# apple/ml-fastvlm

Hardware: AMD Instinct MI355X
Metric: images/sec FastViTHD encode_images @1024x1024 bf16 (higher is better)
Workload: dtype bf16; 1 GPU; BASELINE.json configs[1]: FastViTHD encoder + mlp2x_gelu projector (H=896), batch=32/GPU synthetic 1024x1024 bf16 images in [0,1), seeded synthetic weights, single GPU; global_batch=32, image_size=1024, parallelism=dp1, hip_graph=False, attention_operands=bf16, ffn_precision=auto (calibrated on the benchmark batch), range guard on

## Files before the change

### ml_fastvlm_amd/csrc/gemm.hip

```cpp
#include "fvhd_common.h"
#include "launchers.h"
#include "gemm_layout.h"
#include "rope.h"
#include <stdlib.h>

#define EPI_NONE 0
#define EPI_BIAS 1
#define EPI_BIAS_GELU 2
#define EPI_BIAS_LS_RESID 3
#define EPI_RESID 4
static_assert(FVHD_EPI_SWIGLU_ID == 5 && FVHD_ODT_BF16_ID == FVHD_BF16, "gemm_layout.h ids");
#define EPI_SWIGLU 5

#define EPI_BIAS_ROPE 6

struct RopeArgs {
    const long* pos; const float* table; bf16* kcache; bf16* vcache;
    int M, T, nh, nkv, P; float theta;
};

template <int BK>
FVHD_DEV int lds_off(int row, int ks)
{
    if constexpr (BK == 64) return row * 128 + ((ks ^ ((row >> 1) & 7)) << 4);
    else return row * 64 + ((ks ^ ((0 - (row >> 2)) & 3)) << 4);
}

template <int MF, int NF, int EPI, int ODT, bool ROWMAJOR_ = false>
FVHD_DEV void gemm_epilogue(f32x4 (&acc)[MF][NF], const float* __restrict__ bias, const float* __restrict__ ls, const bf16* resid, void* out,
                            int M, int N, int mw, int nw, int lr, int g)
{
    constexpr int GRP = EpiGrp<NF, EPI, ODT>::value;
#if defined(FVHD_GEMM_EPI_COLMAJOR)
    constexpr bool ROWMAJOR = false;
#elif defined(FVHD_GEMM_EPI_ROWMAJOR)
    constexpr bool ROWMAJOR = ROWMAJOR_;
#else
    constexpr bool ROWMAJOR = ROWMAJOR_ && EPI == EPI_NONE;
#endif
    if constexpr (GRP == 1) {
#pragma unroll
        for (int j = 0; j < NF; ++j) {
            const int n = nw + j * 16 + g * 4;
            if (n >= N) continue;
            f32x4 bv = f32x4{0.f, 0.f, 0.f, 0.f}, lv = f32x4{1.f, 1.f, 1.f, 1.f};
            if constexpr (EPI == EPI_BIAS || EPI == EPI_BIAS_GELU || EPI == EPI_BIAS_LS_RESID) bv = *(const f32x4*)(bias + n);
            if constexpr (EPI == EPI_BIAS_LS_RESID) lv = *(const f32x4*)(ls + n);
#pragma unroll
            for (int i = 0; i < MF; ++i) {
                const int m = mw + i * 16 + lr;
                if (m >= M) continue;
                f32x4 v = acc[i][j] + bv;
                if constexpr (EPI == EPI_SWIGLU) {
                    static_assert(ODT == FVHD_BF16, "SwiGLU writes the bf16 activation");
                    const f32x2 r = {v[0] * sigmoidf_fast(v[0]) * v[1], v[2] * sigmoidf_fast(v[2]) * v[3]};
// ... 172 lines not shown

    const int nk = K / BK;
#pragma unroll
    for (int i = 0; i < A_CH; ++i) ra[i] = *(const u32x4*)(a_src[i]);
#pragma unroll
    for (int i = 0; i < W_CH; ++i) rw[i] = *(const u32x4*)(w_src[i]);

    for (int kt = 0; kt < nk; ++kt) {
        if (kt > 0) __syncthreads();
#pragma unroll
        for (int i = 0; i < A_CH; ++i) *(u32x4*)(ldsA + a_dst[i]) = ra[i];
#pragma unroll
        for (int i = 0; i < W_CH; ++i)
            if (w_dst[i] >= 0) *(u32x4*)(ldsW + w_dst[i]) = rw[i];
        __syncthreads();
        if (kt + 1 < nk) {
            const int ko = (kt + 1) * BK;
#pragma unroll
            for (int i = 0; i < A_CH; ++i) ra[i] = *(const u32x4*)(a_src[i] + ko);
#pragma unroll
            for (int i = 0; i < W_CH; ++i) rw[i] = *(const u32x4*)(w_src[i] + ko);
        }
#pragma unroll
        for (int kk = 0; kk < BK / 32; ++kk) {
            bf16x8 af[MF], wf[NF];
            const int ks = kk * 4 + g;
#pragma unroll
            for (int i = 0; i < MF; ++i) af[i] = *(const bf16x8*)(ldsA + lds_off<BK>(wm * 64 + i * 16 + lr, ks));
#pragma unroll
            for (int j = 0; j < NF; ++j) wf[j] = *(const bf16x8*)(ldsW + lds_off<BK>(wn * 16 * NF + j * 16 + lr, ks));
#pragma unroll
            for (int i = 0; i < MF; ++i)
#pragma unroll
                for (int j = 0; j < NF; ++j)
                    acc[i][j] = __builtin_amdgcn_mfma_f32_16x16x32_bf16(wf[j], af[i], acc[i][j], 0, 0, 0);
        }
    }

    gemm_epilogue<MF, NF, EPI, ODT>(acc, bias, ls, resid, out, M, N, m0 + wm * 64, n0 + wn * 16 * NF, lr, g);
}

template <int BN, int BK = 64, int NWV = 8> struct G2Cfg {
    static constexpr int RS = BK == 64 ? (BN == 256 ? 2 : 3) : (NWV == 4 ? 3 : BN == 256 ? 4 : 6), STAGE = (256 + BN) * BK * 2, LDS = RS * STAGE;
};
template <int BK> FVHD_DEV int lds_swz(int row) { return BK == 64 ? ((row >> 1) & 7) : ((0 - (row >> 2)) & 3); }

FVHD_DEV void glds_piece(unsigned voff, const void* sbase, unsigned m0v)
{
    unsigned keep;
    asm volatile("s_mov_b32 %0, m0\n\ts_mov_b32 m0, %3\n\ts_nop 0\n\tglobal_load_lds_dwordx4 %1, %2\n\ts_mov_b32 m0, %0"
                 : "=&s"(keep) : "v"(voff), "s"(sbase), "s"(m0v) : "memory");
}

template <int EPI, int ODT, int NWV, int BN = 128, int BKT = 64, int ABL = 0>
__global__ __launch_bounds__(64 * NWV, (NWV == 4 && BKT == 32) ? 2 : 1) void gemm256_kernel(
    const bf16* __restrict__ A, const bf16* __restrict__ Wt, const float* __restrict__ bias,
    const float* __restrict__ ls, const bf16* resid, void* out, int M, int N, int K, int tiles_n, int nwg)
{
    constexpr int BM = 256, BK = BKT, WN = BN / 64, WM = NWV / WN, MF = BM / WM / 16, NF = 4, RS = G2Cfg<BN, BK, NWV>::RS, STAGE = G2Cfg<BN, BK, NWV>::STAGE;
    constexpr int RPP = 1024 / (BK * 2), LPR = BK / 8;
    constexpr int PA = (BM / RPP) / NWV, PW = (BN / RPP) / NWV;
    static_assert(WM * WN == NWV && MF * 16 * WM == BM, "wave grid");
    extern __shared__ __attribute__((aligned(16))) char lds2[];
    const int tid = threadIdx.x, lane = tid & 63, wave = __builtin_amdgcn_readfirstlane(tid >> 6);
    const int wm = wave / WN, wn = wave % WN;
    const int lr = lane & 15, g = lane >> 4;
    constexpr int GN = BN == 256 ? 4 : 8;
    const int tiles_m = nwg / tiles_n;
    auto tile_origin = [&](int t, int& m0_, int& n0_) {
        const int L = xcd_remap(t, nwg);
        const int grp = L / (tiles_m * GN), rem = L - grp * tiles_m * GN;
        const int wg = min(GN, tiles_n - grp * GN);
        const int tm = rem / wg, tn = grp * GN + (rem - tm * wg);
        m0_ = tm * BM; n0_ = tn * BN;
    };
    int tile = blockIdx.x, m0, n0;
    tile_origin(tile, m0, n0);

    constexpr int GRP = EpiGrp<NF, EPI, ODT>::value;
    static_assert(GRP == 1 || BK == 64, "the W row permutation is written for 8-row pieces");
    const int rip = lane / LPR;
    unsigned va[2], vw[2];
#pragma unroll
    for (int par = 0; par < 2; ++par) {
        const int sw = lds_swz<BK>(par * RPP + rip);
        va[par] = (unsigned)((rip * K + (((lane % LPR) ^ sw) * 8)) * 2);
        vw[par] = (unsigned)((wpiece_lane_row<GRP>(rip) * K + (((lane % LPR) ^ sw) * 8)) * 2);
    }
    const char* abase = (const char*)(A + (size_t)(m0 + wave * RPP * PA) * K);
    const char* wbase = (const char*)(Wt + (size_t)n0 * K);
    const unsigned lds0 = lds_addr(lds2);
    auto issue = [&](int kt) {
        if constexpr (ABL == 1) return;
        const unsigned st = lds0 + (kt % RS) * STAGE;
        const size_t ko = (size_t)kt * BK * 2;
#pragma unroll
        for (int j = 0; j < PA; ++j) glds_piece(va[(wave * PA + j) & 1], abase + (size_t)j * RPP * K * 2 + ko, st + (wave * PA + j) * 1024);
#pragma unroll
        for (int j = 0; j < PW; ++j) {
            const int pi = wave * PW + j;
            const int wr = GRP == 1 ? pi * RPP : wpiece_row<GRP>(pi);
            glds_piece(vw[pi & 1], wbase + (size_t)wr * K * 2 + ko, st + BM * BK * 2 + pi * 1024);
        }
    };

    const int nk = K / BK;
#pragma unroll
    for (int i = 0; i < RS - 1; ++i)
        if (i < nk) issue(i);
  for (;;) {
    f32x4 acc[MF][NF];
#pragma unroll
    for (int i = 0; i < MF; ++i)
#pragma unroll
        for (int j = 0; j < NF; ++j) acc[i][j] = f32x4{0.f, 0.f, 0.f, 0.f};

    for (int kt = 0; kt < nk; ++kt) {
        {
            const int later = nk - 1 - kt < RS - 2 ? nk - 1 - kt : RS - 2;
            if (later == RS - 2 && RS > 2) asm volatile("s_waitcnt vmcnt(%0)" :: "n"((RS - 2) * (PA + PW)) : "memory");
            else if (RS > 5 && later == 3) asm volatile("s_waitcnt vmcnt(%0)" :: "n"(3 * (PA + PW)) : "memory");
            else if (RS > 4 && later == 2) asm volatile("s_waitcnt vmcnt(%0)" :: "n"(2 * (PA + PW)) : "memory");
            else if (RS > 3 && later == 1) asm volatile("s_waitcnt vmcnt(%0)" :: "n"(1 * (PA + PW)) : "memory");
            else asm volatile("s_waitcnt vmcnt(0)" ::: "memory");
        }
        __syncthreads();
        if (kt + RS - 1 < nk) issue(kt + RS - 1);
        const char* ldsA = lds2 + (kt % RS) * STAGE;
        const char* ldsW = ldsA + BM * BK * 2;
        if constexpr (ABL == 2) continue;
#pragma unroll
        for (int kk = 0; kk < BK / 32; ++kk) {
            bf16x8 af[MF], wf[NF];
            const int ks = kk * 4 + g;
#pragma unroll
            for (int i = 0; i < MF; ++i) af[i] = *(const bf16x8*)(ldsA + lds_off<BK>(wm * 16 * MF + i * 16 + lr, ks));
#pragma unroll
            for (int j = 0; j < NF; ++j) wf[j] = *(const bf16x8*)(ldsW + lds_off<BK>(wn * 64 + j * 16 + lr, ks));
#pragma unroll
            for (int i = 0; i < MF; ++i)
#pragma unroll
                for (int j = 0; j < NF; ++j)
                    acc[i][j] = __builtin_amdgcn_mfma_f32_16x16x32_bf16(wf[j], af[i], acc[i][j], 0, 0, 0);
        }
    }
    const int em0 = m0 + wm * 16 * MF, en0 = n0 + wn * 64;
    tile += gridDim.x;
    const bool more = tile < nwg;
    if (more) {
        __syncthreads();
        tile_origin(tile, m0, n0);
        abase = (const char*)(A + (size_t)(m0 + wave * RPP * PA) * K);
        wbase = (const char*)(Wt + (size_t)n0 * K);
#pragma unroll
        for (int i = 0; i < RS - 1; ++i)
            if (i < nk) issue(i);
    }
    gemm_epilogue<MF, NF, EPI, ODT, true>(acc, bias, ls, resid, out, M, N, em0, en0, lr, g);
    if (!more) break;
  }
}

constexpr int kG128Stages = 4, kG128Stage = (128 + 128) * 64 * 2, kG128Lds = kG128Stages * kG128Stage;
template <int EPI, int ODT>
__global__ __launch_bounds__(256, 1) void gemm128s_kernel(
    const bf16* __restrict__ A, const bf16* __restrict__ Wt, const float* __restrict__ bias,
    const float* __restrict__ ls, const bf16* resid, void* out_, int M, int N, int K, int tiles_n, int nwg, int ldk, RopeArgs rope)
{
    constexpr int BM = 128, BK = 64, MF = 4, NF = 4, RS = kG128Stages, STAGE = kG128Stage, RPP = 8, PA = 4, PW = 4;
    A += (size_t)blockIdx.y * K;
    Wt += (size_t)blockIdx.y * K;
    void* out = ODT == FVHD_F32 ? (void*)((float*)out_ + (size_t)blockIdx.y * M * N) : out_;
    extern __shared__ __attribute__((aligned(16))) char lds2[];
    const int tid = threadIdx.x, lane = tid & 63, wave = __builtin_amdgcn_readfirstlane(tid >> 6);
    const int wm = wave >> 1, wn = wave & 1;
    const int lr = lane & 15, g = lane >> 4;
    const int L = xcd_remap(blockIdx.x, nwg);
    constexpr int GN = 8;
    const int tiles_m = nwg / tiles_n;
    const int grp = L / (tiles_m * GN), rem = L - grp * tiles_m * GN;
    const int wg = min(GN, tiles_n - grp * GN);
    const int tm = rem / wg, tn = grp * GN + (rem - tm * wg);
    const int m0 = tm * BM, n0 = tn * 128;
// ... 10 lines not shown
    const char* abase = (const char*)(A + (size_t)(m0 + wave * RPP * PA) * ldk);
    const char* wbase = (const char*)(Wt + (size_t)n0 * ldk);
    const unsigned lds0 = lds_addr(lds2);
    auto issue = [&](int kt) {
        const unsigned st = lds0 + (kt % RS) * STAGE;
        const size_t ko = (size_t)kt * BK * 2;
#pragma unroll
        for (int j = 0; j < PA; ++j) glds_piece(va[j & 1], abase + (size_t)j * RPP * ldk * 2 + ko, st + (wave * PA + j) * 1024);
#pragma unroll
        for (int j = 0; j < PW; ++j) {
            const int pi = wave * PW + j;
            glds_piece(vw[pi & 1], wbase + (size_t)wpiece_row<GRP>(pi) * ldk * 2 + ko, st + BM * BK * 2 + pi * 1024);
        }
    };

    f32x4 acc[MF][NF];
#pragma unroll
    for (int i = 0; i < MF; ++i)
#pragma unroll
        for (int j = 0; j < NF; ++j) acc[i][j] = f32x4{0.f, 0.f, 0.f, 0.f};

    const int nk = K / BK;
#pragma unroll
    for (int i = 0; i < RS - 1; ++i)
        if (i < nk) issue(i);
    for (int kt = 0; kt < nk; ++kt) {
        const int later = nk - 1 - kt < RS - 2 ? nk - 1 - kt : RS - 2;
        if (later == 2) asm volatile("s_waitcnt vmcnt(%0)" :: "n"(2 * (PA + PW)) : "memory");
        else if (later == 1) asm volatile("s_waitcnt vmcnt(%0)" :: "n"(PA + PW) : "memory");
        else asm volatile("s_waitcnt vmcnt(0)" ::: "memory");
        __syncthreads();
        if (kt + RS - 1 < nk) issue(kt + RS - 1);
        const char* ldsA = lds2 + (kt % RS) * STAGE;
        const char* ldsW = ldsA + BM * BK * 2;
#pragma unroll
        for (int kk = 0; kk < BK / 32; ++kk) {
            bf16x8 af[MF], wf[NF];
            const int ks = kk * 4 + g;
#pragma unroll
            for (int i = 0; i < MF; ++i) af[i] = *(const bf16x8*)(ldsA + lds_off<BK>(wm * 64 + i * 16 + lr, ks));
#pragma unroll
            for (int j = 0; j < NF; ++j) wf[j] = *(const bf16x8*)(ldsW + lds_off<BK>(wn * 64 + j * 16 + lr, ks));
#pragma unroll
            for (int i = 0; i < MF; ++i)
#pragma unroll
                for (int j = 0; j < NF; ++j)
                    acc[i][j] = __builtin_amdgcn_mfma_f32_16x16x32_bf16(wf[j], af[i], acc[i][j], 0, 0, 0);
        }
    }
    if constexpr (EPI == EPI_BIAS_ROPE) gemm_epilogue_rope<MF>(acc, bias, (bf16*)out, rope, M, N, m0 + wm * 64, n0 + wn * 64, lr, g);
    else gemm_epilogue<MF, NF, EPI, ODT, true>(acc, bias, ls, resid, out, M, N, m0 + wm * 64, n0 + wn * 64, lr, g);
}

template <int EPI, int ODT>
__global__ __launch_bounds__(512) void gemm_pp_kernel(
    const bf16* __restrict__ A, const bf16* __restrict__ Wt, const float* __restrict__ bias,
    const float* __restrict__ ls, const bf16* resid, void* out, int M, int N, int K, int tiles_n, int nwg)
{
    constexpr int BM = 256, BN = 256, BK = 64, MF = 8, NF = 4, STAGE = (BM + BN) * 128;
    extern __shared__ __attribute__((aligned(16))) char lds2[];
    const int tid = threadIdx.x, lane = tid & 63, wave = __builtin_amdgcn_readfirstlane(tid >> 6);
    const int grp = wave >> 2, wn = wave & 3;
    const int lr = lane & 15, g = lane >> 4;
    const int L = xcd_remap(blockIdx.x, nwg);
    constexpr int GN = 4;
    const int tiles_m = nwg / tiles_n;
    const int sg = L / (tiles_m * GN), rem = L - sg * tiles_m * GN;
    const int wgw = min(GN, tiles_n - sg * GN);
    const int tm = rem / wgw, tn = sg * GN + (rem - tm * wgw);
    const int m0 = tm * BM, n0 = tn * BN;

    constexpr int GRP = EpiGrp<NF, EPI, ODT>::value;
    const int rip = lane >> 3;
    unsigned vo[2], vwo[2];
#pragma unroll
    for (int par = 0; par < 2; ++par) {
        const int sw = ((par * 8 + rip) >> 1) & 7;
        vo[par] = (unsigned)((rip * K + (((lane & 7) ^ sw) * 8)) * 2);
        vwo[par] = (unsigned)((wpiece_lane_row<GRP>(rip) * K + (((lane & 7) ^ sw) * 8)) * 2);
    }
    const char* abase = (const char*)(A + (size_t)(m0 + wave * 32) * K);
    const char* wbase = (const char*)(Wt + (size_t)n0 * K);
    const unsigned lds0 = lds_addr(lds2);
    auto issue4 = [&](int kt, int which) {
        const unsigned st = lds0 + (kt & 1) * STAGE + (which ? 256 * 128 : 0) + wave * 4096;
        if (which) {
#pragma unroll
            for (int j = 0; j < 4; ++j)
                glds_piece(vwo[j & 1], wbase + (size_t)wpiece_row<GRP>(wave * 4 + j) * K * 2 + (size_t)kt * BK * 2, st + j * 1024);
        } else {
            const char* base = abase + (size_t)kt * BK * 2;
#pragma unroll
            for (int j = 0; j < 4; ++j) glds_piece(vo[j & 1], base + (size_t)j * 8 * K * 2, st + j * 1024);
        }
    };

    f32x4 acc[MF][NF];
#pragma unroll
    for (int i = 0; i < MF; ++i)
#pragma unroll
        for (int j = 0; j < NF; ++j) acc[i][j] = f32x4{0.f, 0.f, 0.f, 0.f};
    bf16x8 af[MF], wf[NF];

    const int nk = K / BK;
    issue4(0, 0); issue4(0, 1);
    if (nk > 1) { issue4(1, 0); issue4(1, 1); }
    asm volatile("s_waitcnt vmcnt(0)" ::: "memory");
    __builtin_amdgcn_s_barrier();
    if (grp == 1) __builtin_amdgcn_s_barrier();

    auto load_phase = [&](int kt, int h) {
        const char* ldsA = lds2 + (kt & 1) * STAGE;
        const char* ldsW = ldsA + 256 * 128;
        const int ks = h * 4 + g;
#pragma unroll
        for (int j = 0; j < NF; ++j) wf[j] = *(const bf16x8*)(ldsW + lds_off<BK>(wn * 64 + j * 16 + lr, ks));
#pragma unroll
        for (int i = 0; i < MF; ++i) af[i] = *(const bf16x8*)(ldsA + lds_off<BK>(grp * 128 + i * 16 + lr, ks));
    };
    auto mfma_phase = [&]() {
        __builtin_amdgcn_s_setprio(1);
#pragma unroll
        for (int i = 0; i < MF; ++i)
#pragma unroll
            for (int j = 0; j < NF; ++j)
                acc[i][j] = __builtin_amdgcn_mfma_f32_16x16x32_bf16(wf[j], af[i], acc[i][j], 0, 0, 0);
        __builtin_amdgcn_s_setprio(0);
    };
#define PP_END(WAIT_VM)                                                                           \
    do {                                                                                          \
        if (WAIT_VM) asm volatile("s_waitcnt vmcnt(0) lgkmcnt(0)" ::: "memory");                  \
        else asm volatile("s_waitcnt lgkmcnt(0)" ::: "memory");                                   \
        __builtin_amdgcn_s_barrier();                                                             \
        __builtin_amdgcn_sched_barrier(0);                                                        \
    } while (0)

    for (int kt = 0; kt < nk; ++kt) {
        const bool d1 = kt >= 1 && kt + 1 < nk, d2 = kt + 2 < nk;
        load_phase(kt, 0);
        if (d1) issue4(kt + 1, grp == 0 ? 0 : 1);
        PP_END(false);
        mfma_phase();
        if (d1 && grp == 0) issue4(kt + 1, 1);
        PP_END(false);
        load_phase(kt, 1);
        PP_END(grp == 1);
        mfma_phase();
        if (d2 && grp == 1) issue4(kt + 2, 0);
        PP_END(grp == 0);
    }
    if (grp == 0) __builtin_amdgcn_s_barrier();
#undef PP_END
    gemm_epilogue<MF, NF, EPI, ODT, true>(acc, bias, ls, resid, out, M, N, m0 + grp * 128, n0 + wn * 64, lr, g);
}

#ifndef FVHD_GEMM_PERSIST_DEFAULT
#define FVHD_GEMM_PERSIST_DEFAULT 0
#endif
static int cu_count()
{
    static int cached[64] = {};
    int dev = 0;
    (void)hipGetDevice(&dev);
    int& n = cached[dev & 63];
    if (n <= 0) {
        int v = 0;
        if (hipDeviceGetAttribute(&v, hipDeviceAttributeMultiprocessorCount, dev) != hipSuccess || v <= 0) v = 256;
        n = v;
    }
    return n;
}

#ifdef FVHD_DEBUG_KNOBS
static int g_gemm_v2 = 1;
extern "C" void fvhd_debug_set_gemm_v2(int on) { g_gemm_v2 = on; }
#else
static constexpr int g_gemm_v2 = 1;
#endif
static const int g_gemm_nf6 = [] { const char* e = getenv("FVHD_GEMM_NF6"); return e ? atoi(e) : 1; }();

template <int EPI, int ODT, int NWV, int BN = 128, int BKT = 64, int ABL = 0>
static hipError_t launch_gemm256(hipStream_t st, const bf16* A, const bf16* Wt, const float* bias, const float* ls,
                                 const bf16* resid, void* out, int M, int N, int K)
{
    static bool attr_set[64] = {};
    int dev = 0;
    (void)hipGetDevice(&dev);
    if (!attr_set[dev & 63]) {
        hipError_t e = hipFuncSetAttribute((const void*)gemm256_kernel<EPI, ODT, NWV, BN, BKT, ABL>, hipFuncAttributeMaxDynamicSharedMemorySize, G2Cfg<BN, BKT, NWV>::LDS);
        if (e != hipSuccess) return e;
        attr_set[dev & 63] = true;
    }
    const int tiles_m = M / 256, tiles_n = N / BN, nwg = tiles_m * tiles_n;
    constexpr int LDSB = G2Cfg<BN, BKT, NWV>::LDS;
    static const int persist = [] { const char* ev = getenv("FVHD_GEMM_PERSIST"); return ev ? atoi(ev) : FVHD_GEMM_PERSIST_DEFAULT; }();
    int grid = nwg;
    if (persist && ABL == 0) {
        const int g8 = cu_count() & ~7;
        if (g8 >= 8 && nwg > g8) grid = g8;
    }
    hipLaunchKernelGGL((gemm256_kernel<EPI, ODT, NWV, BN, BKT, ABL>), dim3(grid), dim3(64 * NWV), LDSB, st, A, Wt, bias, ls, resid, out, M, N, K, tiles_n, nwg);
    return hipGetLastError();
}

template <int EPI, int ODT>
static hipError_t launch_gemm_pp(hipStream_t st, const bf16* A, const bf16* Wt, const float* bias, const float* ls,
                                 const bf16* resid, void* out, int M, int N, int K)
{
    constexpr int LDS = 2 * 512 * 128;
    static bool attr_set[64] = {};
    int dev = 0;
    (void)hipGetDevice(&dev);
    if (!attr_set[dev & 63]) {
        hipError_t e = hipFuncSetAttribute((const void*)gemm_pp_kernel<EPI, ODT>, hipFuncAttributeMaxDynamicSharedMemorySize, LDS);
        if (e != hipSuccess) return e;
        attr_set[dev & 63] = true;
    }
    const int tiles_m = M / 256, tiles_n = N / 256, nwg = tiles_m * tiles_n;
    hipLaunchKernelGGL((gemm_pp_kernel<EPI, ODT>), dim3(nwg), dim3(512), LDS, st, A, Wt, bias, ls, resid, out, M, N, K, tiles_n, nwg);
    return hipGetLastError();
}

static hipError_t dispatch_gemm_pp(hipStream_t st, const bf16* a, const bf16* w, const float* bias, const float* ls, const bf16* r, void* out,
                                   int M, int N, int K, int epi)
{
    switch (epi) {
    case EPI_NONE: return launch_gemm_pp<EPI_NONE, FVHD_BF16>(st, a, w, bias, ls, r, out, M, N, K);
    case EPI_BIAS: return launch_gemm_pp<EPI_BIAS, FVHD_BF16>(st, a, w, bias, ls, r, out, M, N, K);
    case EPI_BIAS_GELU: return launch_gemm_pp<EPI_BIAS_GELU, FVHD_BF16>(st, a, w, bias, ls, r, out, M, N, K);
    case EPI_BIAS_LS_RESID: return launch_gemm_pp<EPI_BIAS_LS_RESID, FVHD_BF16>(st, a, w, bias, ls, r, out, M, N, K);
    case EPI_RESID: return launch_gemm_pp<EPI_RESID, FVHD_BF16>(st, a, w, bias, ls, r, out, M, N, K);
    case EPI_SWIGLU: return launch_gemm_pp<EPI_SWIGLU, FVHD_BF16>(st, a, w, bias, ls, r, out, M, N, K);
    }
    return hipErrorInvalidValue;
}

template <int BN>
static hipError_t dispatch_gemm256(hipStream_t st, const bf16* a, const bf16* w, const float* bias, const float* ls, const bf16* r, void* out,
                                   int M, int N, int K, int epi)
{
    switch (epi) {
    case EPI_NONE: return launch_gemm256<EPI_NONE, FVHD_BF16, 8, BN>(st, a, w, bias, ls, r, out, M, N, K);
    case EPI_BIAS: return launch_gemm256<EPI_BIAS, FVHD_BF16, 8, BN>(st, a, w, bias, ls, r, out, M, N, K);
    case EPI_BIAS_GELU: return launch_gemm256<EPI_BIAS_GELU, FVHD_BF16, 8, BN>(st, a, w, bias, ls, r, out, M, N, K);
    case EPI_BIAS_LS_RESID: return launch_gemm256<EPI_BIAS_LS_RESID, FVHD_BF16, 8, BN>(st, a, w, bias, ls, r, out, M, N, K);
    case EPI_RESID: return launch_gemm256<EPI_RESID, FVHD_BF16, 8, BN>(st, a, w, bias, ls, r, out, M, N, K);
    case EPI_SWIGLU: return launch_gemm256<EPI_SWIGLU, FVHD_BF16, 8, BN>(st, a, w, bias, ls, r, out, M, N, K);
    }
    return hipErrorInvalidValue;
}


template <int EPI, int ODT>
static hipError_t launch_gemm128s(hipStream_t st, const bf16* A, const bf16* Wt, const float* bias, const float* ls, const bf16* resid, void* out,
                                  int M, int N, int K, int splits, int ldk, RopeArgs rope = RopeArgs{})
{
    static bool attr_set[64] = {};
    int dev = 0;
    (void)hipGetDevice(&dev);
    if (!attr_set[dev & 63]) {
        hipError_t e = hipFuncSetAttribute((const void*)gemm128s_kernel<EPI, ODT>, hipFuncAttributeMaxDynamicSharedMemorySize, kG128Lds);
        if (e != hipSuccess) return e;
        attr_set[dev & 63] = true;
    }
    const int tiles_m = M / 128, tiles_n = N / 128, nwg = tiles_m * tiles_n;
    hipLaunchKernelGGL((gemm128s_kernel<EPI, ODT>), dim3(nwg, splits), dim3(256), kG128Lds, st, A, Wt, bias, ls, resid, out, M, N, K, tiles_n, nwg, ldk, rope);
    return hipGetLastError();
}

static hipError_t dispatch_gemm128s(hipStream_t st, const bf16* a, const bf16* w, const float* bias, const float* ls, const bf16* r, void* out,
                                    int M, int N, int K, int epi)
{
    switch (epi) {
    case EPI_NONE: return launch_gemm128s<EPI_NONE, FVHD_BF16>(st, a, w, bias, ls, r, out, M, N, K, 1, K);
    case EPI_BIAS: return launch_gemm128s<EPI_BIAS, FVHD_BF16>(st, a, w, bias, ls, r, out, M, N, K, 1, K);
    case EPI_BIAS_GELU: return launch_gemm128s<EPI_BIAS_GELU, FVHD_BF16>(st, a, w, bias, ls, r, out, M, N, K, 1, K);
    case EPI_BIAS_LS_RESID: return launch_gemm128s<EPI_BIAS_LS_RESID, FVHD_BF16>(st, a, w, bias, ls, r, out, M, N, K, 1, K);
    case EPI_RESID: return launch_gemm128s<EPI_RESID, FVHD_BF16>(st, a, w, bias, ls, r, out, M, N, K, 1, K);
    case EPI_SWIGLU: return launch_gemm128s<EPI_SWIGLU, FVHD_BF16>(st, a, w, bias, ls, r, out, M, N, K, 1, K);
    }
    return hipErrorInvalidValue;
}

#ifndef FVHD_GEMM128S_ROUNDS
#define FVHD_GEMM128S_ROUNDS 1
// ... 122 lines not shown
    return (int)hipGetLastError();
}

extern "C" int fvhd_launch_gemm_splitk_partials(hipStream_t st, const void* A, const void* Wt, float* partial, int M, int N, int K, int splits)
{
    if (M <= 0 || N <= 0 || K <= 0 || splits < 1 || N % 128 || K % (64 * splits) || !partial) return (int)hipErrorInvalidValue;
    return (int)launch_splitk_partials(st, A, Wt, partial, M, N, K, splits);
}

extern "C" int fvhd_launch_gemm_splitk(hipStream_t st, const void* A, const void* Wt, const void* resid, void* out, float* partial,
                                       int M, int N, int K, int splits)
{
    return fvhd_launch_gemm_splitk_norm(st, A, Wt, resid, out, partial, M, N, K, splits, nullptr, nullptr, 0.f);
}

extern "C" int fvhd_gemm_qkv_rope_supported(int Mp, int N, int K, int HD, int nh, int nkv)
{
    if (HD != 64 || Mp <= 0 || nh <= 0 || nkv <= 0 || N != (nh + 2 * nkv) * HD) return 0;
    return take_gemm128s(Mp, N, K, (long)(Mp / 128) * (N / 128)) ? 1 : 0;
}

extern "C" int fvhd_launch_gemm_qkv_rope(hipStream_t st, const void* A, const void* Wt, const float* bias, void* out, int Mp, int N, int K,
                                         const long* pos, const float* table, void* kcache, void* vcache, int M, int T, int nh, int nkv, int HD, int P, float theta)
{
    if (!A || !Wt || !bias || !out || !table || M <= 0 || M > Mp || T <= 0 || P <= 0 || !(theta > 0.f) || (kcache == nullptr) != (vcache == nullptr))
        return (int)hipErrorInvalidValue;
    if (!fvhd_gemm_qkv_rope_supported(Mp, N, K, HD, nh, nkv)) return (int)hipErrorInvalidValue;
    const RopeArgs r{pos, table, (bf16*)kcache, (bf16*)vcache, M, T, nh, nkv, P, theta};
    return (int)launch_gemm128s<EPI_BIAS_ROPE, FVHD_BF16>(st, (const bf16*)A, (const bf16*)Wt, bias, nullptr, nullptr, out, Mp, N, K, 1, K, r);
}

template <int NF, int BK>
static hipError_t dispatch_epi(hipStream_t st, const bf16* A, const bf16* Wt, const float* bias, const float* ls,
                               const bf16* resid, void* out, int M, int N, int K, int epi, int odt)
{
    if (odt == FVHD_BF16) {
        switch (epi) {
        case EPI_NONE: return launch_gemm<NF, BK, EPI_NONE, FVHD_BF16>(st, A, Wt, bias, ls, resid, out, M, N, K);
        case EPI_BIAS: return launch_gemm<NF, BK, EPI_BIAS, FVHD_BF16>(st, A, Wt, bias, ls, resid, out, M, N, K);
        case EPI_BIAS_GELU: return launch_gemm<NF, BK, EPI_BIAS_GELU, FVHD_BF16>(st, A, Wt, bias, ls, resid, out, M, N, K);
        case EPI_BIAS_LS_RESID: return launch_gemm<NF, BK, EPI_BIAS_LS_RESID, FVHD_BF16>(st, A, Wt, bias, ls, resid, out, M, N, K);
        case EPI_RESID: return launch_gemm<NF, BK, EPI_RESID, FVHD_BF16>(st, A, Wt, bias, ls, resid, out, M, N, K);
        case EPI_SWIGLU: return launch_gemm<NF, BK, EPI_SWIGLU, FVHD_BF16>(st, A, Wt, bias, ls, resid, out, M, N, K);
        }
    } else if (epi == EPI_BIAS) {
        if (odt == FVHD_F16) return launch_gemm<NF, BK, EPI_BIAS, FVHD_F16>(st, A, Wt, bias, ls, resid, out, M, N, K);
        if (odt == FVHD_F32) return launch_gemm<NF, BK, EPI_BIAS, FVHD_F32>(st, A, Wt, bias, ls, resid, out, M, N, K);
    } else if (epi == EPI_NONE && odt == FVHD_F32) {
        return launch_gemm<NF, BK, EPI_NONE, FVHD_F32>(st, A, Wt, bias, ls, resid, out, M, N, K);
    }
    return hipErrorInvalidValue;
}

constexpr int kPlanAblate = 100;
static int gemm_plan(int M, int N, int K, int epi, int out_dtype)
{
    if (M <= 0 || N <= 0 || K <= 0 || (K % 32) || (N % 16)) return -1;
    if (out_dtype == FVHD_BF16 ? (epi < EPI_NONE || epi > EPI_SWIGLU)
                               : !((epi == EPI_BIAS && (out_dtype == FVHD_F16 || out_dtype == FVHD_F32)) || (epi == EPI_NONE && out_dtype == FVHD_F32)))
        return -1;
    if (out_dtype == FVHD_BF16 && take_gemm128s(M, N, K, (long)(M / 128) * (N / 128))) return FVHD_GEMM_PLAN_V1S;
    if (g_gemm_v2 && out_dtype == FVHD_BF16 && M % 256 == 0 && N % 128 == 0 && K % 64 == 0 && K >= 128) {
        const long long t128 = (long long)(M / 256) * (N / 128), t256 = N % 256 == 0 ? (long long)(M / 256) * (N / 256) : 0;
#ifdef FVHD_DEBUG_KNOBS
        if ((g_gemm_v2 == 8 || g_gemm_v2 == 9) && t256 > 0 && (epi == EPI_NONE || epi == EPI_BIAS_GELU)) return kPlanAblate;
#endif
        const long long ncu = cu_count();
        const bool use256 = g_gemm_v2 == 3 ? t256 > 0 : (g_gemm_v2 == 1 && N >= 2304 && t256 * 4 >= ncu * 7);
        const long long rounds128 = (t128 + ncu - 1) / ncu;
        const bool full_enough = t128 >= 4 * ncu || t128 * 5 >= rounds128 * ncu * 4;
        const bool use128 = g_gemm_v2 == 2 || (g_gemm_v2 == 1 && ((t128 >= 2 * ncu && full_enough) || (t128 * 2 >= ncu && K >= 3072)));
        if ((g_gemm_v2 == 4 && t256 > 0) || (g_gemm_v2 == 1 && K >= 3072 && t256 * 2 >= ncu)) return FVHD_GEMM_PLAN_PINGPONG;
        if (use256) return FVHD_GEMM_PLAN_256X256;
        if (use128) return FVHD_GEMM_PLAN_256X128;
    }
    const bool nf3 = (N % 128 != 0) && (N % 96 == 0);
    const bool bk64 = (K % 64 == 0);
    if (g_gemm_nf6 && nf3 && bk64 && N % 192 == 0 && epi == EPI_BIAS_GELU && out_dtype == FVHD_BF16 && (long long)((M + 127) / 128) * (N / 192) >= 4ll * cu_count())
        return FVHD_GEMM_PLAN_128X192;
    if (nf3) return bk64 ? FVHD_GEMM_PLAN_V1_NF3_BK64 : FVHD_GEMM_PLAN_V1_NF3_BK32;
    return bk64 ? FVHD_GEMM_PLAN_V1_NF4_BK64 : FVHD_GEMM_PLAN_V1_NF4_BK32;
}

extern "C" int fvhd_gemm_kernel_plan(int M, int N, int K, int epilogue, int out_dtype)
{
    const int p = gemm_plan(M, N, K, epilogue, out_dtype);
    return p == kPlanAblate ? -1 : p;
}

extern "C" int fvhd_launch_gemm(hipStream_t st, const void* A, const void* Wt, const float* bias, const float* ls,
                                const void* resid, void* out, int M, int N, int K, int epi, int out_dtype)
{
    const bf16* a = (const bf16*)A;
    const bf16* w = (const bf16*)Wt;
    const bf16* r = (const bf16*)resid;
    const bool reads_bias = epi == EPI_BIAS || epi == EPI_BIAS_GELU || epi == EPI_BIAS_LS_RESID, reads_resid = epi == EPI_BIAS_LS_RESID || epi == EPI_RESID;
    if (!A || !Wt || !out || (reads_bias && !bias) || (epi == EPI_BIAS_LS_RESID && !ls) || (reads_resid && !resid)) return (int)hipErrorInvalidValue;
    switch (gemm_plan(M, N, K, epi, out_dtype)) {
    case FVHD_GEMM_PLAN_V1S: return (int)dispatch_gemm128s(st, a, w, bias, ls, r, out, M, N, K, epi);
    case FVHD_GEMM_PLAN_PINGPONG: return (int)dispatch_gemm_pp(st, a, w, bias, ls, r, out, M, N, K, epi);
    case FVHD_GEMM_PLAN_256X256: return (int)dispatch_gemm256<256>(st, a, w, bias, ls, r, out, M, N, K, epi);
    case FVHD_GEMM_PLAN_256X128: return (int)dispatch_gemm256<128>(st, a, w, bias, ls, r, out, M, N, K, epi);
    case FVHD_GEMM_PLAN_128X192: return (int)launch_gemm<6, 64, EPI_BIAS_GELU, FVHD_BF16>(st, a, w, bias, ls, r, out, M, N, K);
    case FVHD_GEMM_PLAN_V1_NF3_BK64: return (int)dispatch_epi<3, 64>(st, a, w, bias, ls, r, out, M, N, K, epi, out_dtype);
    case FVHD_GEMM_PLAN_V1_NF3_BK32: return (int)dispatch_epi<3, 32>(st, a, w, bias, ls, r, out, M, N, K, epi, out_dtype);
    case FVHD_GEMM_PLAN_V1_NF4_BK64: return (int)dispatch_epi<4, 64>(st, a, w, bias, ls, r, out, M, N, K, epi, out_dtype);
    case FVHD_GEMM_PLAN_V1_NF4_BK32: return (int)dispatch_epi<4, 32>(st, a, w, bias, ls, r, out, M, N, K, epi, out_dtype);
#ifdef FVHD_DEBUG_KNOBS
    case kPlanAblate:
        if (g_gemm_v2 == 8) return (int)(epi == EPI_NONE ? launch_gemm256<EPI_NONE, FVHD_BF16, 8, 256, 64, 1>(st, a, w, bias, ls, r, out, M, N, K)
                                                          : launch_gemm256<EPI_BIAS_GELU, FVHD_BF16, 8, 256, 64, 1>(st, a, w, bias, ls, r, out, M, N, K));
        return (int)(epi == EPI_NONE ? launch_gemm256<EPI_NONE, FVHD_BF16, 8, 256, 64, 2>(st, a, w, bias, ls, r, out, M, N, K)
                                     : launch_gemm256<EPI_BIAS_GELU, FVHD_BF16, 8, 256, 64, 2>(st, a, w, bias, ls, r, out, M, N, K));
#endif
    }
    return (int)hipErrorInvalidValue;
}
```

Before: 1466 images/sec.

## Replace ping-pong 256x256 GEMM with eight-slot quadrant-phased schedule and route 256x256 plan to it

Rewrites the 256x256 ping-pong GEMM kernel so the tile is split into four half-tile slots (W0, A0, W1, A1) per k-step, double-buffered across eight LDS slots. A table-driven schedule in a new header decides which halves are read, issued and waited on in each of four quadrant phases. The goal is finer overlap of global-to-LDS loads with MFMA work and fewer full vmcnt(0) stalls. The 256x256 plan is also redirected from the older gemm256 kernel to this new kernel, and the debug ablation paths are removed. The cost is more barriers per k-step and a more intricate wait-count scheme that is easy to get wrong.

```diff
diff --git a/ml_fastvlm_amd/csrc/gemm.hip b/ml_fastvlm_amd/csrc/gemm.hip
--- a/ml_fastvlm_amd/csrc/gemm.hip
+++ b/ml_fastvlm_amd/csrc/gemm.hip
@@ -1,6 +1,7 @@
 #include "fvhd_common.h"
 #include "launchers.h"
 #include "gemm_layout.h"
+#include "gemm_sched.h"
 #include "rope.h"
 #include <stdlib.h>
 
@@ -279,7 +280,7 @@
                  : "=&s"(keep) : "v"(voff), "s"(sbase), "s"(m0v) : "memory");
 }
 
-template <int EPI, int ODT, int NWV, int BN = 128, int BKT = 64, int ABL = 0>
+template <int EPI, int ODT, int NWV, int BN = 128, int BKT = 64>
 __global__ __launch_bounds__(64 * NWV, (NWV == 4 && BKT == 32) ? 2 : 1) void gemm256_kernel(
     const bf16* __restrict__ A, const bf16* __restrict__ Wt, const float* __restrict__ bias,
     const float* __restrict__ ls, const bf16* resid, void* out, int M, int N, int K, int tiles_n, int nwg)
@@ -318,7 +319,6 @@
     const char* wbase = (const char*)(Wt + (size_t)n0 * K);
     const unsigned lds0 = lds_addr(lds2);
     auto issue = [&](int kt) {
-        if constexpr (ABL == 1) return;
         const unsigned st = lds0 + (kt % RS) * STAGE;
         const size_t ko = (size_t)kt * BK * 2;
 #pragma unroll
@@ -355,7 +355,6 @@
         if (kt + RS - 1 < nk) issue(kt + RS - 1);
         const char* ldsA = lds2 + (kt % RS) * STAGE;
         const char* ldsW = ldsA + BM * BK * 2;
-        if constexpr (ABL == 2) continue;
 #pragma unroll
         for (int kk = 0; kk < BK / 32; ++kk) {
             bf16x8 af[MF], wf[NF];
@@ -472,12 +471,15 @@
     else gemm_epilogue<MF, NF, EPI, ODT, true>(acc, bias, ls, resid, out, M, N, m0 + wm * 64, n0 + wn * 64, lr, g);
 }
 
+template <int V> struct IntC { static constexpr int value = V; };
 template <int EPI, int ODT>
-__global__ __launch_bounds__(512) void gemm_pp_kernel(
+__global__ __launch_bounds__(512) void gemm8p_kernel(
     const bf16* __restrict__ A, const bf16* __restrict__ Wt, const float* __restrict__ bias,
     const float* __restrict__ ls, const bf16* resid, void* out, int M, int N, int K, int tiles_n, int nwg)
 {
-    constexpr int BM = 256, BN = 256, BK = 64, MF = 8, NF = 4, STAGE = (BM + BN) * 128;
+    namespace S = gemm8;
+    constexpr int BM = 256, BN = 256, BK = 64, MF = 8, NF = 4;
+    static_assert(S::kSlots * S::kSlotBytes == 2 * (BM + BN) * BK * 2 && S::kLoadsPerHalf * 512 * 16 == S::kSlotBytes, "gemm_sched.h geometry");
     extern __shared__ __attribute__((aligned(16))) char lds2[];
     const int tid = threadIdx.x, lane = tid & 63, wave = __builtin_amdgcn_readfirstlane(tid >> 6);
     const int grp = wave >> 2, wn = wave & 3;
@@ -499,78 +501,106 @@
         vo[par] = (unsigned)((rip * K + (((lane & 7) ^ sw) * 8)) * 2);
         vwo[par] = (unsigned)((wpiece_lane_row<GRP>(rip) * K + (((lane & 7) ^ sw) * 8)) * 2);
     }
-    const char* abase = (const char*)(A + (size_t)(m0 + wave * 32) * K);
+    const char* abase = (const char*)(A + (size_t)(m0 + S::a_row(0, 16 * wave)) * K);
     const char* wbase = (const char*)(Wt + (size_t)n0 * K);
     const unsigned lds0 = lds_addr(lds2);
-    auto issue4 = [&](int kt, int which) {
-        const unsigned st = lds0 + (kt & 1) * STAGE + (which ? 256 * 128 : 0) + wave * 4096;
-        if (which) {
-#pragma unroll
-            for (int j = 0; j < 4; ++j)
-                glds_piece(vwo[j & 1], wbase + (size_t)wpiece_row<GRP>(wave * 4 + j) * K * 2 + (size_t)kt * BK * 2, st + j * 1024);
+    auto issue = [&](int half, int t) __attribute__((always_inline)) {
+        const int h = S::half_index(half);
+        const unsigned dst = lds0 + (unsigned)(S::slot_of(half, t) * S::kSlotBytes + wave * 2048);
+        const size_t ko = (size_t)t * BK * 2;
+        if (S::half_is_a(half)) {
+            const char* base = abase + (size_t)(S::a_row(h, 0) - S::a_row(0, 0)) * K * 2 + ko;
+#pragma unroll
+            for (int j = 0; j < 2; ++j) glds_piece(vo[j], base + (size_t)j * 8 * K * 2, dst + j * 1024);
         } else {
-            const char* base = abase + (size_t)kt * BK * 2;
-#pragma unroll
-            for (int j = 0; j < 4; ++j) glds_piece(vo[j & 1], base + (size_t)j * 8 * K * 2, st + j * 1024);
+#pragma unroll
+            for (int j = 0; j < 2; ++j) {
+                const int pi = S::w_row(h, 16 * wave + 8 * j) / 8;
+                glds_piece(vwo[j], wbase + (size_t)wpiece_row<GRP>(pi) * K * 2 + ko, dst + j * 1024);
+            }
         }
     };
+    auto wait_vm = [&](int n) __attribute__((always_inline)) {
+        if (n == 6) asm volatile("s_waitcnt vmcnt(6)" ::: "memory");
+        else if (n == 2) asm volatile("s_waitcnt vmcnt(2)" ::: "memory");
+        else if (n >= 0) asm volatile("s_waitcnt vmcnt(0)" ::: "memory");
+    };
+    static_assert(S::kLoadsPerHalf * S::kInFlight == 6 && S::kLoadsPerHalf == 2, "wait_vm's immediates");
 
     f32x4 acc[MF][NF];
 #pragma unroll
     for (int i = 0; i < MF; ++i)
 #pragma unroll
         for (int j = 0; j < NF; ++j) acc[i][j] = f32x4{0.f, 0.f, 0.f, 0.f};
-    bf16x8 af[MF], wf[NF];
+    bf16x8 af[4][2], wf[NF][2];
+
+    const int key = (lr >> 1) & 7;
+    const int la[2] = {lr * 128 + ((g ^ key) << 4), lr * 128 + (((4 + g) ^ key) << 4)};
+    const char* rdA = lds2 + S::a_frag_row(grp, 0) * 128;
+    const char* rdW = lds2 + S::w_frag_row(wn, 0) * 128;
+    static_assert(S::a_frag_row(0, 1) == 16 && S::w_frag_row(0, 1) == 16 && S::reads_per_half(S::A0) == 8 && S::reads_per_half(S::W0) == 4, "read_half's fragment walk");
+    auto read_half = [&](int half, int par) __attribute__((always_inline)) {
+        const int so = S::slot_of(half, par) * S::kSlotBytes, h = S::half_index(half);
+        if (S::half_is_a(half)) {
+#pragma unroll
+            for (int i = 0; i < 4; ++i)
+#pragma unroll
+                for (int kk = 0; kk < 2; ++kk) af[i][kk] = *(const bf16x8*)(rdA + so + i * 2048 + la[kk]);
+        } else {
+#pragma unroll
+            for (int j = 0; j < 2; ++j)
+#pragma unroll
+                for (int kk = 0; kk < 2; ++kk) wf[2 * h + j][kk] = *(const bf16x8*)(rdW + so + j * 2048 + la[kk]);
+        }
+    };
 
     const int nk = K / BK;
-    issue4(0, 0); issue4(0, 1);
-    if (nk > 1) { issue4(1, 0); issue4(1, 1); }
-    asm volatile("s_waitcnt vmcnt(0)" ::: "memory");
+#pragma unroll
+    for (int i = 0; i < S::kPrologueIssues; ++i)
+        if (S::prologue_issue(i).dt < nk) issue(S::prologue_issue(i).half, S::prologue_issue(i).dt);
+    wait_vm(S::prologue_wait(nk));
     __builtin_amdgcn_s_barrier();
     if (grp == 1) __builtin_amdgcn_s_barrier();
-
-    auto load_phase = [&](int kt, int h) {
-        const char* ldsA = lds2 + (kt & 1) * STAGE;
-        const char* ldsW = ldsA + 256 * 128;
-        const int ks = h * 4 + g;
-#pragma unroll
-        for (int j = 0; j < NF; ++j) wf[j] = *(const bf16x8*)(ldsW + lds_off<BK>(wn * 64 + j * 16 + lr, ks));
-#pragma unroll
-        for (int i = 0; i < MF; ++i) af[i] = *(const bf16x8*)(ldsA + lds_off<BK>(grp * 128 + i * 16 + lr, ks));
+    __builtin_amdgcn_sched_barrier(0);
+
+    auto phase = [&](auto parc, auto qc, int t) __attribute__((always_inline)) {
+        constexpr int PAR = decltype(parc)::value, Q = decltype(qc)::value;
+        constexpr unsigned RD = S::reads_of(Q);
+#pragma unroll
+        for (int half = 0; half < S::kHalves; ++half)
+            if (RD >> half & 1) {
+                read_half(half, PAR);
+                __builtin_amdgcn_sched_barrier(0);
+            }
+        if (S::issues(Q, t, nk)) issue(S::issue_of(Q).half, t + S::issue_of(Q).dt);
+        wait_vm(S::wait_vm(Q, t, nk));
+        if constexpr (S::lgk_before_barrier(Q) == 8) asm volatile("s_waitcnt lgkmcnt(8)" ::: "memory");
+        static_assert(S::lgk_before_barrier(Q) == 8 || S::lgk_before_barrier(Q) < 0, "lgkmcnt immediates");
+        __builtin_amdgcn_sched_barrier(0);
+        __builtin_amdgcn_s_barrier();
+        asm volatile("s_waitcnt lgkmcnt(0)" ::: "memory");
+        __builtin_amdgcn_sched_barrier(0);
+        __builtin_amdgcn_s_setprio(1);
+        constexpr int MH = S::quad_m(Q), NH = S::quad_n(Q);
+#pragma unroll
+        for (int kk = 0; kk < 2; ++kk)
+#pragma unroll
+            for (int i = 0; i < 4; ++i)
+#pragma unroll
+                for (int j = 0; j < 2; ++j)
+                    acc[4 * MH + i][2 * NH + j] = __builtin_amdgcn_mfma_f32_16x16x32_bf16(wf[2 * NH + j][kk], af[i][kk], acc[4 * MH + i][2 * NH + j], 0, 0, 0);
+        __builtin_amdgcn_s_setprio(0);
+        __builtin_amdgcn_sched_barrier(0);
+        __builtin_amdgcn_s_barrier();
+        __builtin_amdgcn_sched_barrier(0);
     };
-    auto mfma_phase = [&]() {
-        __builtin_amdgcn_s_setprio(1);
-#pragma unroll
-        for (int i = 0; i < MF; ++i)
-#pragma unroll
-            for (int j = 0; j < NF; ++j)
-                acc[i][j] = __builtin_amdgcn_mfma_f32_16x16x32_bf16(wf[j], af[i], acc[i][j], 0, 0, 0);
-        __builtin_amdgcn_s_setprio(0);
-    };
-#define PP_END(WAIT_VM)                                                                           \
-    do {                                                                                          \
-        if (WAIT_VM) asm volatile("s_waitcnt vmcnt(0) lgkmcnt(0)" ::: "memory");                  \
-        else asm volatile("s_waitcnt lgkmcnt(0)" ::: "memory");                                   \
-        __builtin_amdgcn_s_barrier();                                                             \
-        __builtin_amdgcn_sched_barrier(0);                                                        \
-    } while (0)
-
-    for (int kt = 0; kt < nk; ++kt) {
-        const bool d1 = kt >= 1 && kt + 1 < nk, d2 = kt + 2 < nk;
-        load_phase(kt, 0);
-        if (d1) issue4(kt + 1, grp == 0 ? 0 : 1);
-        PP_END(false);
-        mfma_phase();
-        if (d1 && grp == 0) issue4(kt + 1, 1);
-        PP_END(false);
-        load_phase(kt, 1);
-        PP_END(grp == 1);
-        mfma_phase();
-        if (d2 && grp == 1) issue4(kt + 2, 0);
-        PP_END(grp == 0);
+    for (int t = 0; t < nk; t += 2) {
+        phase(IntC<0>{}, IntC<0>{}, t); phase(IntC<0>{}, IntC<1>{}, t); phase(IntC<0>{}, IntC<2>{}, t); phase(IntC<0>{}, IntC<3>{}, t);
+        if (t + 1 < nk) {
+            phase(IntC<1>{}, IntC<0>{}, t + 1); phase(IntC<1>{}, IntC<1>{}, t + 1); phase(IntC<1>{}, IntC<2>{}, t + 1); phase(IntC<1>{}, IntC<3>{}, t + 1);
+        }
     }
     if (grp == 0) __builtin_amdgcn_s_barrier();
-#undef PP_END
     gemm_epilogue<MF, NF, EPI, ODT, true>(acc, bias, ls, resid, out, M, N, m0 + grp * 128, n0 + wn * 64, lr, g);
 }
 
@@ -599,7 +629,7 @@
 #endif
 static const int g_gemm_nf6 = [] { const char* e = getenv("FVHD_GEMM_NF6"); return e ? atoi(e) : 1; }();
 
-template <int EPI, int ODT, int NWV, int BN = 128, int BKT = 64, int ABL = 0>
+template <int EPI, int ODT, int NWV, int BN = 128, int BKT = 64>
 static hipError_t launch_gemm256(hipStream_t st, const bf16* A, const bf16* Wt, const float* bias, const float* ls,
                                  const bf16* resid, void* out, int M, int N, int K)
 {
@@ -607,7 +637,7 @@
     int dev = 0;
     (void)hipGetDevice(&dev);
     if (!attr_set[dev & 63]) {
-        hipError_t e = hipFuncSetAttribute((const void*)gemm256_kernel<EPI, ODT, NWV, BN, BKT, ABL>, hipFuncAttributeMaxDynamicSharedMemorySize, G2Cfg<BN, BKT, NWV>::LDS);
+        hipError_t e = hipFuncSetAttribute((const void*)gemm256_kernel<EPI, ODT, NWV, BN, BKT>, hipFuncAttributeMaxDynamicSharedMemorySize, G2Cfg<BN, BKT, NWV>::LDS);
         if (e != hipSuccess) return e;
         attr_set[dev & 63] = true;
     }
@@ -615,42 +645,43 @@
     constexpr int LDSB = G2Cfg<BN, BKT, NWV>::LDS;
     static const int persist = [] { const char* ev = getenv("FVHD_GEMM_PERSIST"); return ev ? atoi(ev) : FVHD_GEMM_PERSIST_DEFAULT; }();
     int grid = nwg;
-    if (persist && ABL == 0) {
+    if (persist) {
         const int g8 = cu_count() & ~7;
         if (g8 >= 8 && nwg > g8) grid = g8;
     }
-    hipLaunchKernelGGL((gemm256_kernel<EPI, ODT, NWV, BN, BKT, ABL>), dim3(grid), dim3(64 * NWV), LDSB, st, A, Wt, bias, ls, resid, out, M, N, K, tiles_n, nwg);
+    hipLaunchKernelGGL((gemm256_kernel<EPI, ODT, NWV, BN, BKT>), dim3(grid), dim3(64 * NWV), LDSB, st, A, Wt, bias, ls, resid, out, M, N, K, tiles_n, nwg);
     return hipGetLastError();
 }
 
 template <int EPI, int ODT>
-static hipError_t launch_gemm_pp(hipStream_t st, const bf16* A, const bf16* Wt, const float* bias, const float* ls,
-                                 const bf16* resid, void* out, int M, int N, int K)
-{
-    constexpr int LDS = 2 * 512 * 128;
+static hipError_t launch_gemm8p(hipStream_t st, const bf16* A, const bf16* Wt, const float* bias, const float* ls,
+                                const bf16* resid, void* out, int M, int N, int K)
+{
+    constexpr int LDS = gemm8::kSlots * gemm8::kSlotBytes;
+    if (M % 256 || N % 256 || K % 64 || K < 128) return hipErrorInvalidValue;
     static bool attr_set[64] = {};
     int dev = 0;
     (void)hipGetDevice(&dev);
     if (!attr_set[dev & 63]) {
-        hipError_t e = hipFuncSetAttribute((const void*)gemm_pp_kernel<EPI, ODT>, hipFuncAttributeMaxDynamicSharedMemorySize, LDS);
+        hipError_t e = hipFuncSetAttribute((const void*)gemm8p_kernel<EPI, ODT>, hipFuncAttributeMaxDynamicSharedMemorySize, LDS);
         if (e != hipSuccess) return e;
         attr_set[dev & 63] = true;
     }
     const int tiles_m = M / 256, tiles_n = N / 256, nwg = tiles_m * tiles_n;
-    hipLaunchKernelGGL((gemm_pp_kernel<EPI, ODT>), dim3(nwg), dim3(512), LDS, st, A, Wt, bias, ls, resid, out, M, N, K, tiles_n, nwg);
+    hipLaunchKernelGGL((gemm8p_kernel<EPI, ODT>), dim3(nwg), dim3(512), LDS, st, A, Wt, bias, ls, resid, out, M, N, K, tiles_n, nwg);
     return hipGetLastError();
 }
 
-static hipError_t dispatch_gemm_pp(hipStream_t st, const bf16* a, const bf16* w, const float* bias, const float* ls, const bf16* r, void* out,
-                                   int M, int N, int K, int epi)
+static hipError_t dispatch_gemm8p(hipStream_t st, const bf16* a, const bf16* w, const float* bias, const float* ls, const bf16* r, void* out,
+                                  int M, int N, int K, int epi)
 {
     switch (epi) {
-    case EPI_NONE: return launch_gemm_pp<EPI_NONE, FVHD_BF16>(st, a, w, bias, ls, r, out, M, N, K);
-    case EPI_BIAS: return launch_gemm_pp<EPI_BIAS, FVHD_BF16>(st, a, w, bias, ls, r, out, M, N, K);
-    case EPI_BIAS_GELU: return launch_gemm_pp<EPI_BIAS_GELU, FVHD_BF16>(st, a, w, bias, ls, r, out, M, N, K);
-    case EPI_BIAS_LS_RESID: return launch_gemm_pp<EPI_BIAS_LS_RESID, FVHD_BF16>(st, a, w, bias, ls, r, out, M, N, K);
-    case EPI_RESID: return launch_gemm_pp<EPI_RESID, FVHD_BF16>(st, a, w, bias, ls, r, out, M, N, K);
-    case EPI_SWIGLU: return launch_gemm_pp<EPI_SWIGLU, FVHD_BF16>(st, a, w, bias, ls, r, out, M, N, K);
+    case EPI_NONE: return launch_gemm8p<EPI_NONE, FVHD_BF16>(st, a, w, bias, ls, r, out, M, N, K);
+    case EPI_BIAS: return launch_gemm8p<EPI_BIAS, FVHD_BF16>(st, a, w, bias, ls, r, out, M, N, K);
+    case EPI_BIAS_GELU: return launch_gemm8p<EPI_BIAS_GELU, FVHD_BF16>(st, a, w, bias, ls, r, out, M, N, K);
+    case EPI_BIAS_LS_RESID: return launch_gemm8p<EPI_BIAS_LS_RESID, FVHD_BF16>(st, a, w, bias, ls, r, out, M, N, K);
+    case EPI_RESID: return launch_gemm8p<EPI_RESID, FVHD_BF16>(st, a, w, bias, ls, r, out, M, N, K);
+    case EPI_SWIGLU: return launch_gemm8p<EPI_SWIGLU, FVHD_BF16>(st, a, w, bias, ls, r, out, M, N, K);
     }
     return hipErrorInvalidValue;
 }
@@ -879,7 +910,6 @@
     return hipErrorInvalidValue;
 }
 
-constexpr int kPlanAblate = 100;
 static int gemm_plan(int M, int N, int K, int epi, int out_dtype)
 {
     if (M <= 0 || N <= 0 || K <= 0 || (K % 32) || (N % 16)) return -1;
@@ -889,9 +919,6 @@
     if (out_dtype == FVHD_BF16 && take_gemm128s(M, N, K, (long)(M / 128) * (N / 128))) return FVHD_GEMM_PLAN_V1S;
     if (g_gemm_v2 && out_dtype == FVHD_BF16 && M % 256 == 0 && N % 128 == 0 && K % 64 == 0 && K >= 128) {
         const long long t128 = (long long)(M / 256) * (N / 128), t256 = N % 256 == 0 ? (long long)(M / 256) * (N / 256) : 0;
-#ifdef FVHD_DEBUG_KNOBS
-        if ((g_gemm_v2 == 8 || g_gemm_v2 == 9) && t256 > 0 && (epi == EPI_NONE || epi == EPI_BIAS_GELU)) return kPlanAblate;
-#endif
         const long long ncu = cu_count();
         const bool use256 = g_gemm_v2 == 3 ? t256 > 0 : (g_gemm_v2 == 1 && N >= 2304 && t256 * 4 >= ncu * 7);
         const long long rounds128 = (t128 + ncu - 1) / ncu;
@@ -911,8 +938,7 @@
 
 extern "C" int fvhd_gemm_kernel_plan(int M, int N, int K, int epilogue, int out_dtype)
 {
-    const int p = gemm_plan(M, N, K, epilogue, out_dtype);
-    return p == kPlanAblate ? -1 : p;
+    return gemm_plan(M, N, K, epilogue, out_dtype);
 }
 
 extern "C" int fvhd_launch_gemm(hipStream_t st, const void* A, const void* Wt, const float* bias, const float* ls,
@@ -925,21 +951,14 @@
     if (!A || !Wt || !out || (reads_bias && !bias) || (epi == EPI_BIAS_LS_RESID && !ls) || (reads_resid && !resid)) return (int)hipErrorInvalidValue;
     switch (gemm_plan(M, N, K, epi, out_dtype)) {
     case FVHD_GEMM_PLAN_V1S: return (int)dispatch_gemm128s(st, a, w, bias, ls, r, out, M, N, K, epi);
-    case FVHD_GEMM_PLAN_PINGPONG: return (int)dispatch_gemm_pp(st, a, w, bias, ls, r, out, M, N, K, epi);
-    case FVHD_GEMM_PLAN_256X256: return (int)dispatch_gemm256<256>(st, a, w, bias, ls, r, out, M, N, K, epi);
+    case FVHD_GEMM_PLAN_PINGPONG:
+    case FVHD_GEMM_PLAN_256X256: return (int)dispatch_gemm8p(st, a, w, bias, ls, r, out, M, N, K, epi);
     case FVHD_GEMM_PLAN_256X128: return (int)dispatch_gemm256<128>(st, a, w, bias, ls, r, out, M, N, K, epi);
     case FVHD_GEMM_PLAN_128X192: return (int)launch_gemm<6, 64, EPI_BIAS_GELU, FVHD_BF16>(st, a, w, bias, ls, r, out, M, N, K);
     case FVHD_GEMM_PLAN_V1_NF3_BK64: return (int)dispatch_epi<3, 64>(st, a, w, bias, ls, r, out, M, N, K, epi, out_dtype);
     case FVHD_GEMM_PLAN_V1_NF3_BK32: return (int)dispatch_epi<3, 32>(st, a, w, bias, ls, r, out, M, N, K, epi, out_dtype);
     case FVHD_GEMM_PLAN_V1_NF4_BK64: return (int)dispatch_epi<4, 64>(st, a, w, bias, ls, r, out, M, N, K, epi, out_dtype);
     case FVHD_GEMM_PLAN_V1_NF4_BK32: return (int)dispatch_epi<4, 32>(st, a, w, bias, ls, r, out, M, N, K, epi, out_dtype);
-#ifdef FVHD_DEBUG_KNOBS
-    case kPlanAblate:
-        if (g_gemm_v2 == 8) return (int)(epi == EPI_NONE ? launch_gemm256<EPI_NONE, FVHD_BF16, 8, 256, 64, 1>(st, a, w, bias, ls, r, out, M, N, K)
-                                                          : launch_gemm256<EPI_BIAS_GELU, FVHD_BF16, 8, 256, 64, 1>(st, a, w, bias, ls, r, out, M, N, K));
-        return (int)(epi == EPI_NONE ? launch_gemm256<EPI_NONE, FVHD_BF16, 8, 256, 64, 2>(st, a, w, bias, ls, r, out, M, N, K)
-                                     : launch_gemm256<EPI_BIAS_GELU, FVHD_BF16, 8, 256, 64, 2>(st, a, w, bias, ls, r, out, M, N, K));
-#endif
     }
     return (int)hipErrorInvalidValue;
 }
diff --git a/ml_fastvlm_amd/csrc/gemm_sched.h b/ml_fastvlm_amd/csrc/gemm_sched.h
--- /dev/null
+++ b/ml_fastvlm_amd/csrc/gemm_sched.h
@@ -0,0 +1,42 @@
+#pragma once
+
+namespace gemm8 {
+
+enum Half : int { W0 = 0, A0 = 1, W1 = 2, A1 = 3 };
+constexpr int kHalves = 4, kPhases = 4, kSlots = 8, kSlotBytes = 16384;
+constexpr int kLoadsPerHalf = 2;
+constexpr int kInFlight = 3;
+
+struct Issue { int half, dt; };
+
+constexpr bool half_is_a(int half) { return (half & 1) != 0; }
+constexpr int half_index(int half) { return half >> 1; }
+constexpr int slot_of(int half, int t) { return kHalves * (t & 1) + half; }
+constexpr int a_row(int h, int r) { return 128 * (r / 64) + 64 * h + r % 64; }
+constexpr int w_row(int h, int r) { return 64 * (r / 32) + 32 * h + r % 32; }
+constexpr int a_frag_row(int grp, int i) { return 64 * grp + 16 * i; }
+constexpr int w_frag_row(int wn, int j) { return 32 * wn + 16 * j; }
+constexpr int reads_per_half(int half) { return half_is_a(half) ? 8 : 4; }
+
+constexpr unsigned reads_of(int q) { return q == 0 ? (1u << W0 | 1u << A0) : q == 1 ? 1u << W1 : q == 2 ? 1u << A1 : 0u; }
+constexpr int quad_m(int q) { return q >> 1; }
+constexpr int quad_n(int q) { return q & 1; }
+constexpr int lgk_before_barrier(int q) { return q == 0 ? 8 : -1; }
+constexpr unsigned lgk_retires(int q) { return q == 0 ? 1u << W0 : 0u; }
+constexpr Issue issue_of(int q) { return q == 0 ? Issue{A1, 1} : q == 1 ? Issue{W0, 2} : q == 2 ? Issue{A0, 2} : Issue{W1, 2}; }
+constexpr bool issues(int q, int t, int nk) { return t + issue_of(q).dt < nk; }
+constexpr int wait_vm(int q, int t, int nk)
+{
+    if (q == 3) return t + 2 < nk ? kLoadsPerHalf * kInFlight : t + 1 < nk ? kLoadsPerHalf : -1;
+    if (q == 1) return (t + 1 == nk && nk > 1) ? 0 : -1;
+    return -1;
+}
+constexpr bool wait_is_steady(int q, int t, int nk) { return q == 3 && t + 2 < nk; }
+
+constexpr int kPrologueIssues = 7;
+constexpr Issue prologue_issue(int i) { return i < kHalves ? Issue{i, 0} : Issue{i - kHalves, 1}; }
+constexpr int prologue_wait(int nk) { return nk > 1 ? kLoadsPerHalf * kInFlight : 0; }
+
+constexpr int tick_of_phase(int grp, int p) { return 2 * p + grp; }
+
+}
```

Result: no change. 1479 images/sec (median of 6 runs) (+0.9%).
